# OmerShubi/DL_VQA

Hardware: AMD Instinct MI355X
Metric: VQA samples/sec (train step) (higher is better)
Workload: dtype f32; 1 GPU; VqaNet train step (fwd+softCE+bwd+Adam), batch 256/GPU, 224x224 images, 14-token questions, 1000-way head, train mode; global_batch=256, image_size=224, answers=1000, vocab=5000, parallelism=dp1

## Files before the change

dl_vqa_amd/_lib.py:

```python
from __future__ import annotations

import ctypes as C
import os

import torch

_HERE = os.path.dirname(os.path.abspath(__file__))
LIB_PATH = os.environ.get("VQA_LIB", os.path.join(_HERE, "libvqa_hip.so"))
HEADER_PATH = os.path.join(os.path.dirname(_HERE), "include", "vqa_hip.h")


def header_abi_version() -> int:
    import re
    with open(HEADER_PATH) as f:
        m = re.search(r"^#define\s+VQA_ABI_VERSION\s+(\d+)", f.read(), flags=re.M)
    if not m:
        raise VqaHipError(f"{HEADER_PATH}: no VQA_ABI_VERSION")
    return int(m.group(1))


f32p = C.c_void_p
u8p = C.c_void_p
i64p = C.c_void_p
i32, i64, f32, u64, vp = C.c_int, C.c_int64, C.c_float, C.c_uint64, C.c_void_p

PROTOTYPES = {
    "vqa_abi_version": (i32, []),
    "vqa_last_error": (C.c_char_p, []),
    "vqa_device_ok": (i32, []),
    "vqa_reload_knobs": (i32, []),
    "vqa_prof_arm": (i32, [i32, i32]),
    "vqa_prof_arm_mask": (i32, [C.c_uint32, i32]),
    "vqa_prof_read": (i32, [C.POINTER(i32), C.POINTER(f32)]),
    "vqa_prof_read_groups": (i32, [C.POINTER(i32), C.POINTER(i32), C.POINTER(i32), C.POINTER(f32), i32]),
    "vqa_gemm_workspace_bytes": (i64, [i32, i32, i32]),
    "vqa_gemm": (i32, [f32p, i64, i32, f32p, i64, i32, f32p, i64, i32, i32, i32, f32p, f32p,
                       f32p, i64, i32, i32, i32, i32, f32p, f32p, i64, i32, vp]),
    "vqa_gemm_x3": (i32, [f32p, i64, i32, f32p, i64, i32, f32p, i64, i32, i32, i32, f32p, f32p,
                       f32p, i64, i32, i32, i32, i32, f32p, f32p, i64, i32, vp]),
    "vqa_gemm_x3_workspace_bytes": (i64, [i32, i32, i32]),
    "vqa_nchw_to_nhwc4": (i32, [f32p, f32p, i32, i32, i32, i32, vp]),
    "vqa_conv_pack_weights": (i32, [f32p, f32p, f32p, i32, i32, i32, vp]),
    "vqa_conv3x3_relu_pool_fwd": (i32, [f32p, f32p, f32p, f32p, u8p, i32, i32, i32, i32, i32, i32, i32, vp]),
    "vqa_conv3x3_dgrad": (i32, [f32p, u8p, f32p, f32p, i32, i32, i32, i32, i32, i32, i32, vp]),
    "vqa_conv3x3_wgrad_workspace_bytes": (i64, [i32, i32, i32, i32, i32, i32]),
    "vqa_conv3x3_wgrad": (i32, [f32p, f32p, u8p, f32p, f32p, i32, i32, i32, i32, i32, i32, i32,
                                f32p, i64, i32, vp]),
    "vqa_convk_pack_weights": (i32, [f32p, f32p, i32, i32, i32, i32, vp]),
    "vqa_convk_unpack_wgrad": (i32, [f32p, f32p, i32, i32, i32, i32, vp]),
    "vqa_convk_im2col": (i32, [f32p, f32p, i32, i32, i32, i32, i32, i32, vp]),
    "vqa_convk_relu_pool": (i32, [f32p, f32p, u8p, i32, i32, i32, i32, vp]),
    "vqa_convk_route": (i32, [f32p, u8p, f32p, i32, i32, i32, i32, vp]),
    "vqa_convk_col2im": (i32, [f32p, f32p, i32, i32, i32, i32, i32, i32, vp]),
    "vqa_conv3x3_x3_supported": (i32, [i32, i32, i32, i32, i32]),
    "vqa_x3_split": (i32, [f32p, vp, vp, vp, i64, vp]),
    "vqa_x3_pack": (i32, [f32p, vp, i64, vp]),
    "vqa_x3_pack_pooled_grad_workspace_bytes": (i64, [i32]),
    "vqa_x3_pack_pooled_grad": (i32, [f32p, u8p, vp, f32p, i64, i32, f32p, i64, vp]),
    "vqa_conv3x3_relu_pool_fwd_x3": (i32, [vp, i32, vp, f32p, vp, i32, u8p, i32, i32, i32, i32, i32, i32, i32, vp]),
    "vqa_conv3x3_dgrad_x3": (i32, [vp, i32, u8p, vp, f32p, i32, i32, i32, i32, i32, i32, i32, vp]),
    "vqa_conv3x3_wgrad_x3_workspace_bytes": (i64, [i32, i32, i32, i32, i32, i32]),
    "vqa_conv3x3_wgrad_x3": (i32, [vp, i32, f32p, vp, u8p, f32p, f32p, i32, i32, i32, i32, i32, i32, i32,
                                   f32p, i64, i32, vp]),
    "vqa_conv0_supported": (i32, [i32, i32, i32, i32, i32]),
    "vqa_conv0_relu_pool_fwd": (i32, [vp, i32, f32p, f32p, vp, i32, u8p, i32, i32, i32, i32, i32, vp]),
    "vqa_conv0_wgrad_workspace_bytes": (i64, [i32]),
    "vqa_conv0_wgrad": (i32, [vp, i32, f32p, u8p, f32p, f32p, i32, i32, i32, i32, i32, f32p, i64, vp]),
    "vqa_conv0_wgrad_bf16": (i32, [vp, i32, vp, u8p, f32p, f32p, i32, i32, i32, i32, i32, f32p, i64, vp]),
    "vqa_conv0_dgrad_supported": (i32, [i32, i32, i32, i32, i32]),
    "vqa_conv0_dgrad": (i32, [vp, i32, u8p, f32p, vp, i32, i32, i32, i32, i32, i32, i32, vp]),
# ... 185 lines not shown
```

dl_vqa_amd/build.py:

```python
from __future__ import annotations

import os
import subprocess
import sys
from concurrent.futures import ThreadPoolExecutor

HERE = os.path.dirname(os.path.abspath(__file__))
CSRC = os.path.join(HERE, "csrc")
LIB = os.path.join(HERE, "libvqa_hip.so")
SOURCES = ([("gemm.hip", f"_p{k}", [f"-DVQA_GEMM_PART={k}"]) for k in (2, 3, 4, 5)]
           + [("gemm_x3.hip", f"_p{k}", [f"-DVQA_GEMM_PART={k}"]) for k in (1, 2, 3, 4)]
           + ["bf16.hip", ("gemm.hip", "_p1", ["-DVQA_GEMM_PART=1"]), "conv.hip", "conv_x3.hip", "conv_bf16.hip", "conv_patch_bf16.hip", "conv_patch_f32.hip", "gemm_tall_bf16.hip", "gemm.hip",
              "gemm_x3.hip", "runtime.hip", "conv0.hip", "conv0_dgrad.hip", "lstm.hip", "elementwise.hip", "conv_generic.hip", "att_score.hip", "att_apply.hip", "occlusion.hip", "faithfulness.hip", "lstm_occl.hip", "topk.hip", "preprocess.hip",
              "gather.hip", "adam.hip"])
HEADERS = ["common.hpp", "cache_load.hpp", "occl_core.hpp", "gemm_core.hpp", "gemm_epilogue.hpp", "gemm_host.hpp", "bf16_core.hpp", "x3_core.hpp", "conv_device.inc", "conv_host.inc", "conv_bf16.inc", os.path.join("..", "..", "include", "vqa_hip.h")]
FLAGS = ["-O3", "--offload-arch=gfx950", "-fPIC", "-std=c++17", "-Wno-unused-result"]


def _hipcc() -> str:
    for cand in (os.environ.get("HIPCC"), "/opt/rocm/bin/hipcc", "hipcc"):
        if cand and (os.path.isabs(cand) and os.path.exists(cand) or not os.path.isabs(cand)):
            return cand
    return "hipcc"


def _stale(target: str, deps) -> bool:
    if not os.path.exists(target):
        return True
    t = os.path.getmtime(target)
    return any(os.path.getmtime(d) > t for d in deps if os.path.exists(d))


def _deps(src: str, seen=None) -> list:
    import re
    seen = set() if seen is None else seen
    out = []
    try:
        text = open(src).read()
# ... 43 lines not shown
```

dl_vqa_amd/csrc/common.hpp:

```cpp
#pragma once
#include <hip/hip_runtime.h>
#include <stdint.h>
#include <stdio.h>
#include <string.h>

#include <type_traits>

#include "../../include/vqa_hip.h"

namespace vqa {

void set_error(const char* fmt, ...);
int check_hip(hipError_t e, const char* what);

#define VQA_REQUIRE(cond, ...)                 \
  do {                                         \
    if (!(cond)) {                             \
      ::vqa::set_error(__VA_ARGS__);           \
      return VQA_ERR_INVALID;                  \
    }                                          \
  } while (0)

int ensure_dyn_smem(const void* kernel, int bytes, const char* what);
template <class K>
// ... 28 lines not shown
}
template <class F>
static int with_int14(int v, F&& f) {
  switch (v) {
    case 1: return f(std::integral_constant<int, 1>{});
    case 2: return f(std::integral_constant<int, 2>{});
    case 3: return f(std::integral_constant<int, 3>{});
    default: return f(std::integral_constant<int, 4>{});
  }
}

template <class... P>
static inline uintptr_t ptr_bits(const P*... p) { return (uintptr_t{0} | ... | reinterpret_cast<uintptr_t>(p)); }

static inline float keep_scale(float p) { return p > 0.f ? 1.0f / (1.0f - p) : 1.0f; }

struct Knobs {
  int split_target;
  int big_tiles;
  int persistent;
  int weight_stationary;
  int wgrad_192;
  int wgrad_384;
  int conv_chunk;
  int tall_bm;
};
const Knobs& knobs();

void set_launch_tag(int tag);
struct ProfScope {
  int id;
  hipStream_t s;
  bool on;
  ProfScope(int id_, hipStream_t s_);
  ~ProfScope();
};

__device__ __forceinline__ int xcd_swizzle(int bid, int nwg) {
  const int xcd = bid & 7, q = nwg >> 3, r = nwg & 7;
  const int base = (xcd < r) ? xcd * (q + 1) : r * (q + 1) + (xcd - r) * q;
  return base + (bid >> 3);
}

__device__ __forceinline__ uint32_t mix32(uint32_t x) {
  x ^= x >> 16; x *= 0x7feb352dU; x ^= x >> 15; x *= 0x846ca68bU; x ^= x >> 16;
  return x;
// ... 60 lines not shown
```

dl_vqa_amd/csrc/conv.hip:

```cpp
#include "bf16_core.hpp"

namespace vqa {

#include "conv_device.inc"
#include "conv_host.inc"

using Cfg128 = TileCfg<128, 128, 2, 2>;
using Cfg128x64 = TileCfg<128, 64, 2, 2>;
#ifndef VQA_BIG_PF
#define VQA_BIG_PF 0
#endif
using Cfg256x128 = TileCfg<256, 128, 4, 2, 4, VQA_BIG_PF>;
using Cfg256x64 = TileCfg<256, 64, 4, 2, 4, VQA_BIG_PF>;
using Cfg64 = TileCfg<64, 64, 2, 2>;
#ifndef VQA_WGRAD_PF
#define VQA_WGRAD_PF 3
#endif
using Cfg96x128 = TileCfg<96, 128, 1, 4, 4, VQA_WGRAD_PF>;
using Cfg128W = TileCfg<128, 128, 2, 2, 4, VQA_WGRAD_PF>;
#ifndef VQA_W192_PF
#define VQA_W192_PF 3
#endif
using Cfg192x128W = TileCfg<192, 128, 2, 4, 4, VQA_W192_PF>;
using Cfg384x128W = TileCfg<384, 128, 4, 2, 4, 2>;
// ... 40 lines not shown
  const int big = (KI >= 128 && g.Co >= 128) ? 1 : 0;
  int bm = !big ? 64 : ((KI + 95) / 96 * 96 < (KI + 127) / 128 * 128 ? 96 : 128);
  {
    const int w192 = knobs().wgrad_192, w384 = knobs().wgrad_384;
    const bool can = big && KI % 192 == 0 && g.CiP % BK == 0 && g.Co % BK == 0 && 2 * g.Wp >= BK;
    if (can && (w192 >= 0 ? w192 == 1 : bm == 96)) bm = 192;
    if (can && KI % 384 == 0 && w192 != 1 && (w384 >= 0 ? w384 == 1 : true)) bm = 384;
  }
  WgradPlanF p{plan_splits(g, bm, big ? 128 : 64, BK, bm >= 192 ? 256 : 512), big, bm};
  p.bias_parts = p.splits;
  return p;
}

template <class Cfg, bool U>
static int launch_wgrad(const float* x, const float* dp, const uint8_t* am, float* slab, float* bias_slab,
                        const ConvGeom& g, const WgradPlan& p, hipStream_t s) {
  using SL = SmemLayout<Cfg, false, false>;
  WgradGeom wg{g.H, g.W, g.CiP, g.Hp, g.Wp, g.Co, g.stride, p.Mtot};
  typename WgradA<Cfg::NVA, Cfg::LT, U>::Params pa{x, wg, p.KI};
  typename WgradB<Cfg::NVB, Cfg::LT, U>::Params pb{dp, am, wg};
  return launch_kernel(conv_wgrad_kernel<Cfg, U>, {"attr(conv_wgrad)", "conv_wgrad launch"},
                       p.tiles_m * p.tiles_n * p.splits, Cfg::THREADS, SL::BYTES, s, pa, pb, slab, bias_slab, p.tiles_m,
                       p.tiles_n, p.nk, p.ks_per_split);
}

}

using namespace vqa;

extern "C" {

int vqa_nchw_to_nhwc4(const float* x, float* y, int B, int C, int H, int W, vqa_stream_t stream) {
  VQA_REQUIRE(x && y && C >= 1 && C <= 4, "vqa_nchw_to_nhwc4: C=%d must be 1..4", C);
  const int64_t HW = (int64_t)H * W, total = (int64_t)B * HW;
  int blocks = (int)((total + 255) / 256);
  if (blocks > 8192) blocks = 8192;
  hipLaunchKernelGGL(nchw_to_nhwc4_kernel, dim3(blocks), dim3(256), 0, (hipStream_t)stream, x, y, C, HW, total);
  return check_hip(hipGetLastError(), "nchw_to_nhwc4 launch");
}

int vqa_conv_pack_weights(const float* w, float* wf, float* wd, int Co, int Ci, int CiP, vqa_stream_t stream) {
  VQA_REQUIRE(w && wf && Ci <= CiP && CiP % 4 == 0, "vqa_conv_pack_weights: bad args Ci=%d CiP=%d", Ci, CiP);
  const int total = 9 * CiP * Co;
  hipLaunchKernelGGL(pack_weights_kernel, dim3((total + 255) / 256), dim3(256), 0, (hipStream_t)stream, w, wf, wd,
                     Co, Ci, CiP);
  return check_hip(hipGetLastError(), "pack_weights launch");
// ... 37 lines not shown
int64_t vqa_conv3x3_wgrad_workspace_bytes(int B, int H, int W, int CiP, int Co, int stride) {
  if (no_windows(B, H, W, stride)) return 0;
  const ConvWalk w{"vqa_conv3x3_wgrad", B, H, W, CiP, Co, stride, batch_chunk(B, H, W, CiP, Co, stride)};
  return slab_bytes(w, count_slabs(w, plan_wgrad));
}

int vqa_conv3x3_wgrad(const float* x, const float* dpooled, const uint8_t* argmax, float* dw, float* dbias, int B,
                      int H, int W, int CiP, int Ci, int Co, int stride, float* workspace, int64_t workspace_bytes,
                      int tag, vqa_stream_t stream) {
  VQA_REQUIRE(x && dpooled && argmax && dw && dbias && workspace && B > 0, "vqa_conv3x3_wgrad: null pointer");
  VQA_REQUIRE(Ci >= 1 && Ci <= CiP, "vqa_conv3x3_wgrad: Ci=%d CiP=%d", Ci, CiP);
  const ConvWalk w{"vqa_conv3x3_wgrad", B, H, W, CiP, Co, stride, batch_chunk(B, H, W, CiP, Co, stride)};
  hipStream_t s = (hipStream_t)stream;
  return wgrad_walk(
      w, plan_wgrad, 0, workspace, workspace_bytes, dw, Ci, tag, s,
      [&](const ConvChunk& c, const WgradPlanF& p, float* slab, float* bias_slab) {
        auto go = [&](auto cfg, auto uni) {
          return launch_wgrad<decltype(cfg), decltype(uni)::value>(x + c.xo, dpooled + c.po, argmax + c.po, slab, bias_slab,
                                                                   c.g, p, s);
        };
        auto go_uni = [&](auto cfg) {
          return with_flag(CiP % BK == 0 && Co % BK == 0 && 2 * c.g.Wp >= BK, [&](auto uni) { return go(cfg, uni); });
        };
        return p.bm == 384   ? go(Cfg384x128W{}, Flag<true>{})
               : p.bm == 192 ? go(Cfg192x128W{}, Flag<true>{})
               : p.bm == 96  ? go_uni(Cfg96x128{})
               : p.big       ? go_uni(Cfg128W{})
                             : go_uni(Cfg64{});
      },
      [&](const float* bias_rows, int n) { return reduce_bias_rows(bias_rows, dbias, n, Co, s); });
}

}

#ifdef VQA_DIAG
extern "C" int vqa_diag_read(unsigned long long* out8) {
  unsigned long long z[4] = {0, 0, 0, 0};
  hipDeviceSynchronize();
  if (hipMemcpyFromSymbol(out8, HIP_SYMBOL(vqa::vqa_diag_buf), sizeof(z)) != hipSuccess) return 1;
  if (hipMemcpyFromSymbol(out8 + 4, HIP_SYMBOL(vqa::vqa_diag_ld), sizeof(z)) != hipSuccess) return 1;
  if (hipMemcpyToSymbol(HIP_SYMBOL(vqa::vqa_diag_ld), z, sizeof(z)) != hipSuccess) return 1;
  return hipMemcpyToSymbol(HIP_SYMBOL(vqa::vqa_diag_buf), z, sizeof(z)) == hipSuccess ? 0 : 1;
}
#endif
```

dl_vqa_amd/csrc/conv_device.inc:

```
#ifdef VQA_EXP_NOAM
#define AM_LOAD(...) 0u
#else
#define AM_LOAD(...) buf_load4(__VA_ARGS__)
#endif

struct ConvGeom {
  int B, H, W, CiP, Co, stride, Ho, Wo, Hp, Wp;
};
static ConvGeom make_geom(int B, int H, int W, int CiP, int Co, int stride) {
  ConvGeom g{B, H, W, CiP, Co, stride, 0, 0, 0, 0};
  g.Ho = (H - 3) / stride + 1;
  g.Wo = (W - 3) / stride + 1;
  g.Hp = g.Ho / 2;
  g.Wp = g.Wo / 2;
  return g;
}

struct TapCursor {
  int tap, ch, C;
  __device__ __forceinline__ void init(int k, int C_) { C = C_; tap = k / C_; ch = k - tap * C_; }
  __device__ __forceinline__ void advance() {
    ch += BK;
    while (ch >= C) { ch -= C; ++tap; }
  }
};

// ... 521 lines not shown
    if (rc.yo + 1 == rc.Ho2 && n1 < BK) l1 += fix_img;
    const uint32_t off = kr < n1 ? lp0 : l1;
    if ((ks + 1) * BK <= q.g.Mtot) {
#pragma unroll
      for (int p = 0; p < NV; ++p) r.v[p] = buf_load16(rs, off, base + su[p]);
    } else {
      const uint32_t o2 = rc.m0 + kr < q.g.Mtot ? off + base : BUF_OOB;
#pragma unroll
      for (int p = 0; p < NV; ++p) r.v[p] = buf_load16(rs, o2, su[p]);
    }
    rc.advance();
  }
  __device__ __forceinline__ void finish(const Raw& r, float4 (&o)[NV]) const {
#pragma unroll
    for (int p = 0; p < NV; ++p) o[p] = r.v[p];
  }
};

template <int NV, int LT>
struct WgradB<NV, LT, true> {
  struct Params { const float* dp; const uint8_t* am; WgradGeom g; };
  struct Raw { float4 d[NV]; uint32_t id[NV]; uint32_t j; };
  static constexpr bool kTypeR = false;
  Params q;
  uint32_t lw0, lwE;
  uint32_t j0, win;
  int kr, n0, hw;
  RowCursor rc;
  __device__ __forceinline__ void init(const Params& q_, int n0_, int tid, int ks0) {
    q = q_; n0 = n0_;
    kr = StageMap<LT>::c_krow(tid);
    hw = __builtin_amdgcn_readfirstlane(tid >> 8);
    rc.init(ks0 * BK, q.g.Hp, q.g.Wp);
    win = (uint32_t)q.g.Co * 4u;
    lw0 = (uint32_t)(kr >> 1) * win + 16u * (uint32_t)(tid & 7);
    lwE = lw0 - (uint32_t)q.g.Wp * win;
    j0 = (uint32_t)(kr & 1);
  }
  __device__ __forceinline__ void issue(int ks, Raw& r) {
    const __amdgpu_buffer_rsrc_t rd = buf_rsrc(q.dp + n0), ra = buf_rsrc(q.am + n0, BUF_OOB >> 2);
    const int n1 = rc.Wo2 - rc.xs;
    const bool odd = rc.yo & 1;
    const int R = rc.b * rc.Ho2 + rc.yo;
    const uint32_t base = (uint32_t)((R >> 1) * q.g.Wp + (rc.xs >> 1)) * win;
    const bool second = kr >= n1;
    uint32_t off = (second && !odd ? lwE : lw0) + base;
// ... 35 lines not shown
  float cs[Cfg::TN];
#pragma unroll
  for (int j = 0; j < Cfg::TN; ++j) cs[j] = 0.f;
  if (!gemm_mainloop<Cfg, AL, BL>(
          [&](AL& al, BL& bl) {
            al.init(pa, m0, loader_tid<Cfg>(), ks0);
            bl.init(pb, n0, loader_tid<Cfg>(), ks0);
          },
          [](AL&, BL&) {}, acc, ks0, ks1, pa.g.Mtot, smem, (tc.mt == 0 && wm == 0) ? cs : nullptr))
    return;
  if (tc.mt == 0 && wm == 0) {
#pragma unroll
    for (int j = 0; j < Cfg::TN; ++j) {
      const float v = cs[j] + __shfl_xor(cs[j], 32, 64);
      const int col = n0 + acc_col<Cfg>(wn, j, lane);
      if (lane < 32 && col < pa.g.Co) bias_slab[(int64_t)split * pa.g.Co + col] = v;
    }
  }
  const int Co = pa.g.Co;
  float* out = slab + (int64_t)split * pa.KI * Co;
  store_acc_tiles<Cfg>(acc, out, Co, pa.KI, Co, m0, n0, wm, wn, lane);
}

static __global__ __launch_bounds__(256) void wgrad_reduce_kernel(const float* slab, float* dw, int splits, int KI, int CiP,
                                                           int Ci, int Co) {
  __shared__ float part[4][64];
  const int lane = threadIdx.x & 63, grp = threadIdx.x >> 6;
  const int src = blockIdx.x * 64 + lane;
  const int total = KI * Co;
  float v = 0.f;
  if (src < total)
    for (int s = grp; s < splits; s += 4) v += slab[(int64_t)s * total + src];
  part[grp][lane] = v;
  __syncthreads();
  if (grp == 0 && src < total) {
    v = (part[0][lane] + part[1][lane]) + (part[2][lane] + part[3][lane]);
    const int co = src % Co;
    const int t = src / Co;
    const int ci = t % CiP;
    const int tap = t / CiP;
    if (ci < Ci) dw[((int64_t)co * Ci + ci) * 9 + tap] = v;
  }
}

static __global__ __launch_bounds__(256) void wgrad_bias_reduce_kernel(const float* bias_slab, float* dbias, int parts, int Co) {
  __shared__ float part[8][32];
// ... 41 lines not shown
```

dl_vqa_amd/csrc/conv_patch_bf16.hip:

```cpp
#include "bf16_core.hpp"
#include <stdlib.h>

namespace vqa {

#ifdef VQA_PCONV_DIAG
#define PC_DBG(bit) (P.dbg & (bit))
#else
#define PC_DBG(bit) false
#endif

constexpr int PC_RS = 40;
constexpr int PC_TX = 32;

template <int WM_>
struct PcCfg {
  static constexpr int WM = WM_, WN = 8 / WM_;
  static constexpr int TY = 4 * WM;
  static constexpr int NSLAB = 64 * WN;
  static constexpr int NT = NSLAB / 32;
  static constexpr int PROWS = TY + 2;
  static constexpr int PATCH_BYTES = ((PROWS * PC_RS * 32 + 1023) / 1024) * 1024;
  static constexpr int PATCH_INSTR = PATCH_BYTES / 1024;
  static constexpr int PK = (PATCH_INSTR + 7) / 8;
  static constexpr int W_BYTES = 9 * NT * 1024;
// ... 6 lines not shown
  static constexpr int LDS_ALL = LDS + 8 * SCR;
  template <int EPI> static constexpr int nstores() { return EPI == 0 ? 8 : EPI == 1 ? 12 : 16; }
};

struct PcParams {
  const char* x;
  const char* x_end;
  const char* wimg;
  const float* bias;
  void* out;
  uint8_t* amax;
  const char* am_in;
  int Hq, Wq;
  int B, H, W, Cin, N;
  int Hc, Wc;
  int Hp, Wp;
  int tiles_y, tiles_x, ntiles;
  int nslabs, nslices;
  int dbg;
};

typedef __attribute__((address_space(3))) void lds_void;

typedef unsigned int pc_rsrc_t __attribute__((ext_vector_type(4)));
__device__ __forceinline__ pc_rsrc_t pc_rsrc(const void* base, uint32_t bytes = 0xffff0000u) {
  const uint64_t a = (uint64_t)base;
  pc_rsrc_t r;
  r.x = __builtin_amdgcn_readfirstlane((uint32_t)a);
  r.y = __builtin_amdgcn_readfirstlane((uint32_t)(a >> 32) & 0xffffu);
  r.z = __builtin_amdgcn_readfirstlane(bytes);
  r.w = 0x00020000u;
  return r;
}
__device__ __forceinline__ void lds_dma16(pc_rsrc_t r, const void* lds_dst, uint32_t voff, uint32_t soff) {
  const uint32_t m0v = __builtin_amdgcn_readfirstlane((uint32_t)(uintptr_t)(__attribute__((address_space(3))) const char*)lds_dst);
  uint32_t keep;
  asm volatile("s_nop 4\n\ts_mov_b32 %0, m0\n\ts_mov_b32 m0, %1\n\ts_nop 0\n\tbuffer_load_dwordx4 %2, %3, %4 offen lds\n\ts_mov_b32 m0, %0"
               : "=&s"(keep) : "s"(m0v), "v"(voff), "s"(r), "s"(soff) : "memory");
}

struct PcTile {
  int img, ty, tx;
  __device__ __forceinline__ void decode(int s, int tiles_y, int tiles_x) {
    const int per = tiles_y * tiles_x;
    img = s / per;
    const int rem = s - img * per;
    ty = rem / tiles_x;
    tx = rem - ty * tiles_x;
  }
  __device__ __forceinline__ void advance(const PcTile& d, int tiles_y, int tiles_x) {
    tx += d.tx;
    if (tx >= tiles_x) { tx -= tiles_x; ++ty; }
    ty += d.ty;
    if (ty >= tiles_y) { ty -= tiles_y; ++img; }
    img += d.img;
  }
};

__device__ __forceinline__ float4 pc_route8(float4 d, uint2 id, uint32_t j) {
  const uint32_t jj = j * 0x01010101u;
  auto bytemask = [&](uint32_t w) {
    const uint32_t q = w ^ jj;
// ... 764 lines not shown
```

dl_vqa_amd/csrc/gemm_core.hpp:

```cpp
#pragma once
#include <type_traits>
#include "common.hpp"

namespace vqa {

typedef float f32x16 __attribute__((ext_vector_type(16)));

#ifdef VQA_DIAG
static __device__ unsigned long long vqa_diag_buf[4];
static __device__ unsigned long long vqa_diag_ld[4];
#endif

#ifndef VQA_PRIO_MFMA
#define VQA_PRIO_MFMA 3
#endif
#ifndef VQA_EARLY_BARRIER
#define VQA_EARLY_BARRIER 2
#endif
#ifndef VQA_PF128
#define VQA_PF128 2
#endif
#ifndef VQA_PRIO_LOADER
#define VQA_PRIO_LOADER 0
#endif

// ... 274 lines not shown
        __syncthreads();
#elif defined(VQA_EXP_STORE_ONLY)
        stage_store_one<Cfg, AL, true>(al, rawA[d], As0 + nxt * SL::ABUF, ltid);
        stage_store_one<Cfg, BL, false>(bl, rawB[d], Bs0 + nxt * SL::BBUF, ltid);
        __syncthreads();
#else
        stage_store_one<Cfg, AL, true>(al, rawA[d], As0 + nxt * SL::ABUF, ltid);
        al.issue(ks + d + 1 + D, rawA[d]);
        stage_store_one<Cfg, BL, false>(bl, rawB[d], Bs0 + nxt * SL::BBUF, ltid);
        bl.issue(ks + d + 1 + D, rawB[d]);
        __syncthreads();
#endif
      }
    }
  }
#ifdef VQA_DIAG
  if ((threadIdx.x & 63) == 0) {
    atomicAdd(&vqa_diag_ld[0], t_st); atomicAdd(&vqa_diag_ld[1], t_is); atomicAdd(&vqa_diag_ld[2], t_ba);
    atomicAdd(&vqa_diag_ld[3], 1ULL);
  }
#endif
}

template <class Cfg, bool AR, bool BR, bool SHORT_TAIL, bool CS = false>
__device__ __forceinline__ void mfma_loop(f32x16 (&acc)[Cfg::TM][Cfg::TN], int ks0, int ks1, int Ktot,
                                          const float* smem, float* cs = nullptr) {
  using SL = SmemLayout<Cfg, AR, BR>;
  const int lane = threadIdx.x & 63, wave = threadIdx.x >> 6;
  const int wm = wave / Cfg::WAVES_N, wn = wave % Cfg::WAVES_N;
  const float* const As0 = smem;
  const float* const Bs0 = smem + 2 * SL::ABUF;
  __builtin_amdgcn_s_setprio(VQA_PRIO_MFMA);
#ifdef VQA_DIAG
  unsigned long long t_mma = 0, t_bar = 0;
  const unsigned long long t_begin = __builtin_amdgcn_s_memtime();
#endif
  __syncthreads();
  for (int ks = ks0; ks < ks1; ++ks) {
    const int cur = (ks - ks0) & 1;
    const float* const Ac = As0 + cur * SL::ABUF;
    const float* const Bc = Bs0 + cur * SL::BBUF;
#ifdef VQA_DIAG
    const unsigned long long t0 = __builtin_amdgcn_s_memtime();
#endif
#ifndef VQA_EXP_SKIP_MFMA
    if (SHORT_TAIL && Ktot - ks * BK <= 8) mma_steps<Cfg, AR, BR, 1, CS>(Ac, Bc, acc, wm, wn, lane, cs);
    else mma_steps<Cfg, AR, BR, 4, CS>(Ac, Bc, acc, wm, wn, lane, cs);
#endif
#ifdef VQA_DIAG
    const unsigned long long t1 = __builtin_amdgcn_s_memtime();
#endif
    __syncthreads();
#ifdef VQA_DIAG
    const unsigned long long t2 = __builtin_amdgcn_s_memtime();
    t_mma += t1 - t0; t_bar += t2 - t1;
#endif
  }
#ifdef VQA_DIAG
  if (lane == 0) {
    atomicAdd(&vqa_diag_buf[0], t_mma); atomicAdd(&vqa_diag_buf[1], t_bar); atomicAdd(&vqa_diag_buf[2], 1ULL);
    atomicAdd(&vqa_diag_buf[3], __builtin_amdgcn_s_memtime() - t_begin);
  }
#endif
}

template <class Cfg, bool AR, bool BR, bool CS>
__device__ __forceinline__ void mfma_loop_eb(f32x16 (&acc)[Cfg::TM][Cfg::TN], int ks0, int ks1, const float* smem,
                                             float* cs) {
  using SL = SmemLayout<Cfg, AR, BR>;
  const int lane = threadIdx.x & 63, wave = threadIdx.x >> 6;
  const int wm = wave / Cfg::WAVES_N, wn = wave % Cfg::WAVES_N;
  const int l31 = lane & 31, h = lane >> 5;
  constexpr int CSA = LdsImage<Cfg::BM>::CS, CSB = LdsImage<Cfg::BN>::CS;
  const float* const As0 = smem + (AR ? (wm * Cfg::WM + l31) * LDS_RS + 4 * h : 4 * h * CSA + wm * Cfg::WM + l31);
  const float* const Bs0 = smem + 2 * SL::ABUF + (BR ? (wn * Cfg::WN + l31) * LDS_RS + 4 * h : 4 * h * CSB + wn * Cfg::WN + l31);
  constexpr bool EB2 = Cfg::TM * Cfg::TN == 1 && VQA_EARLY_BARRIER >= 2;
  float a[EB2 ? 4 : 2][4][Cfg::TM], b[EB2 ? 4 : 2][4][Cfg::TN];
  auto fetch = [&](const float* ap, const float* bp, int t, int buf) {
#pragma unroll
    for (int i = 0; i < Cfg::TM; ++i) {
      if (AR) {
        const float4 v = *reinterpret_cast<const float4*>(ap + 32 * i * LDS_RS + 8 * t);
        a[buf][0][i] = v.x; a[buf][1][i] = v.y; a[buf][2][i] = v.z; a[buf][3][i] = v.w;
      } else {
#pragma unroll
        for (int q = 0; q < 4; ++q) a[buf][q][i] = ap[(8 * t + q) * CSA + 32 * i];
      }
    }
#pragma unroll
    for (int j = 0; j < Cfg::TN; ++j) {
      if (BR) {
        const float4 v = *reinterpret_cast<const float4*>(bp + 32 * j * LDS_RS + 8 * t);
        b[buf][0][j] = v.x; b[buf][1][j] = v.y; b[buf][2][j] = v.z; b[buf][3][j] = v.w;
      } else {
#pragma unroll
        for (int q = 0; q < 4; ++q) b[buf][q][j] = bp[(8 * t + q) * CSB + 32 * j];
      }
    }
  };
// ... 24 lines not shown
      const float* const An = As0 + (cur ^ 1) * SL::ABUF;
      const float* const Bn = Bs0 + (cur ^ 1) * SL::BBUF;
      fetch(Ac, Bc, 2, 2);
      __builtin_amdgcn_sched_barrier(0);
      mma(0);
      __builtin_amdgcn_sched_barrier(0);
      fetch(Ac, Bc, 3, 3);
      __builtin_amdgcn_sched_barrier(0);
      mma(1);
      __builtin_amdgcn_sched_barrier(0);
      __syncthreads();
      if (ks + 1 < ks1) fetch(An, Bn, 0, 0);
      __builtin_amdgcn_sched_barrier(0);
      mma(2);
      __builtin_amdgcn_sched_barrier(0);
      if (ks + 1 < ks1) fetch(An, Bn, 1, 1);
      __builtin_amdgcn_sched_barrier(0);
      mma(3);
      __builtin_amdgcn_sched_barrier(0);
    }
    return;
  }
  fetch(As0, Bs0, 0, 0);
  for (int ks = ks0; ks < ks1; ++ks) {
    const int cur = (ks - ks0) & 1;
    const float* const Ac = As0 + cur * SL::ABUF;
    const float* const Bc = Bs0 + cur * SL::BBUF;
#pragma unroll
    for (int t = 0; t < 3; ++t) {
      fetch(Ac, Bc, t + 1, (t + 1) & 1);
      __builtin_amdgcn_sched_barrier(0);
      mma(t & 1);
      __builtin_amdgcn_sched_barrier(0);
    }
    __syncthreads();
    if (ks + 1 < ks1) fetch(As0 + (cur ^ 1) * SL::ABUF, Bs0 + (cur ^ 1) * SL::BBUF, 0, 0);
    __builtin_amdgcn_sched_barrier(0);
    mma(1);
    __builtin_amdgcn_sched_barrier(0);
  }
}

template <class Cfg, class AL, class BL, bool SHORT_TAIL = false, class Init, class Done>
__device__ __forceinline__ bool gemm_mainloop(Init&& init, Done&& done, f32x16 (&acc)[Cfg::TM][Cfg::TN], int ks0,
                                              int ks1, int Ktot, float* smem, float* cs = nullptr) {
  if (is_loader_wave<Cfg>()) {
    AL al; BL bl;
    init(al, bl);
    loader_loop<Cfg>(al, bl, ks0, ks1, smem);
    done(al, bl);
    return false;
  }
#if VQA_EARLY_BARRIER && !defined(VQA_DIAG) && !defined(VQA_EXP_SKIP_MFMA)
  if (!SHORT_TAIL) {
    if (cs) mfma_loop_eb<Cfg, AL::kTypeR, BL::kTypeR, true>(acc, ks0, ks1, smem, cs);
    else mfma_loop_eb<Cfg, AL::kTypeR, BL::kTypeR, false>(acc, ks0, ks1, smem, nullptr);
    return true;
  }
#endif
  if (cs) mfma_loop<Cfg, AL::kTypeR, BL::kTypeR, SHORT_TAIL, true>(acc, ks0, ks1, Ktot, smem, cs);
  else mfma_loop<Cfg, AL::kTypeR, BL::kTypeR, SHORT_TAIL, false>(acc, ks0, ks1, Ktot, smem);
  return true;
}
// ... 160 lines not shown
```

dl_vqa_amd/csrc/runtime.hip:

```cpp
#include <stdarg.h>
#include <stdlib.h>

#include <map>
#include <mutex>
#include <set>
#include <utility>
#include <vector>

#include "gemm_host.hpp"

namespace vqa {

static thread_local char g_err[512] = "";
void set_error(const char* fmt, ...) {
  va_list ap;
  va_start(ap, fmt);
  vsnprintf(g_err, sizeof(g_err), fmt, ap);
  va_end(ap);
}
int check_hip(hipError_t e, const char* what) {
  if (e == hipSuccess) return VQA_OK;
  set_error("%s: %s", what, hipGetErrorString(e));
  return VQA_ERR_HIP;
}
// ... 39 lines not shown
  if (per_cu < 1) {
    set_error("gemm_persistent: the kernel does not fit a CU (occupancy query says %d workgroups)", per_cu);
    return -1;
  }
  const int slots = cus * (per_cu < planned_per_cu ? per_cu : planned_per_cu);
  cache[key] = slots;
  return slots;
}

static std::mutex g_knob_mu;
static Knobs g_knobs;
static bool g_knobs_read = false;
static int env_int(const char* name) {
  const char* e = getenv(name);
  return (e && *e) ? atoi(e) : -1;
}
static void read_knobs_locked() {
  g_knobs.split_target = env_int("VQA_SPLIT_TARGET");
  g_knobs.big_tiles = env_int("VQA_BIG_TILES");
  g_knobs.persistent = env_int("VQA_PERSISTENT");
  g_knobs.weight_stationary = env_int("VQA_WEIGHT_STATIONARY");
  g_knobs.wgrad_192 = env_int("VQA_WGRAD_192");
  g_knobs.wgrad_384 = env_int("VQA_WGRAD_384");
  g_knobs.conv_chunk = env_int("VQA_CONV_CHUNK");
  g_knobs.tall_bm = env_int("VQA_TALL_BM");
  g_knobs_read = true;
}
const Knobs& knobs() {
  std::lock_guard<std::mutex> lk(g_knob_mu);
  if (!g_knobs_read) read_knobs_locked();
  return g_knobs;
}

static std::mutex g_prof_mu;
static uint32_t g_prof_mask = 0;
static int g_prof_tag = -1;
static std::vector<std::pair<hipEvent_t, hipEvent_t>> g_prof_ev;
static std::vector<std::pair<int, int>> g_prof_key;
static thread_local int g_launch_tag = -1;
void set_launch_tag(int tag) { g_launch_tag = tag; }

ProfScope::ProfScope(int id_, hipStream_t s_) : id(id_), s(s_), on(false) {
  if (g_prof_mask == 0) return;
  std::lock_guard<std::mutex> lk(g_prof_mu);
  if (!((g_prof_mask >> id) & 1u) || (g_prof_tag >= 0 && g_prof_tag != g_launch_tag)) return;
  hipStreamCaptureStatus cap = hipStreamCaptureStatusNone;
// ... 154 lines not shown
```

include/vqa_hip.h:

```cpp
#ifndef VQA_HIP_H
#define VQA_HIP_H

#include <stdint.h>

#ifdef __cplusplus
extern "C" {
#endif

#define VQA_ABI_VERSION 9

#define VQA_OK 0
#define VQA_ERR_INVALID 1
#define VQA_ERR_HIP 2
#define VQA_ERR_WORKSPACE 3

typedef void* vqa_stream_t;

int vqa_abi_version(void);
const char* vqa_last_error(void);
int vqa_device_ok(void);

int vqa_reload_knobs(void);

enum {
// ... 16 lines not shown
int vqa_prof_arm(int kernel_id, int tag);
int vqa_prof_arm_mask(uint32_t mask, int tag);
int vqa_prof_read(int* launches, float* total_ms);
int vqa_prof_read_groups(int* ids, int* tags, int* launches, float* total_ms, int cap);

int64_t vqa_gemm_workspace_bytes(int M, int N, int K);
int vqa_gemm(const float* A, int64_t lda, int transA, const float* B, int64_t ldb, int transB,
             float* C, int64_t ldc, int M, int N, int K, const float* bias1, const float* bias2,
             const float* rowgroup, int64_t rg_ld, int rg_div, int rg_op, int relu, int accumulate,
             float* aux ,
             float* workspace, int64_t workspace_bytes, int tag, vqa_stream_t stream);

int vqa_nchw_to_nhwc4(const float* x_nchw, float* y_nhwc, int B, int C, int H, int W, vqa_stream_t stream);
int vqa_conv_pack_weights(const float* w, float* wf, float* wd, int Co, int Ci, int CiP, vqa_stream_t stream);
int vqa_conv3x3_relu_pool_fwd(const float* x, const float* wf, const float* bias, float* pooled,
                              uint8_t* argmax, int B, int H, int W, int CiP, int Co, int stride,
                              int tag, vqa_stream_t stream);
int vqa_conv3x3_dgrad(const float* dpooled, const uint8_t* argmax, const float* wd, float* dx, int B,
                      int H, int W, int CiP, int Co, int stride, int tag, vqa_stream_t stream);
int64_t vqa_conv3x3_wgrad_workspace_bytes(int B, int H, int W, int CiP, int Co, int stride);
int vqa_conv3x3_wgrad(const float* x, const float* dpooled, const uint8_t* argmax, float* dw,
                      float* dbias, int B, int H, int W, int CiP, int Ci, int Co, int stride,
                      float* workspace, int64_t workspace_bytes, int tag, vqa_stream_t stream);

int vqa_convk_pack_weights(const float* w, float* wk, int Co, int Ci, int CiP, int ks, vqa_stream_t stream);
int vqa_convk_unpack_wgrad(const float* dwk, float* dw, int Co, int Ci, int CiP, int ks, vqa_stream_t stream);
int vqa_convk_im2col(const float* x, float* cols, int B, int H, int W, int CiP, int ks, int stride, vqa_stream_t stream);
int vqa_convk_relu_pool(const float* y, float* pooled, uint8_t* argmax, int B, int Ho, int Wo, int Co, vqa_stream_t stream);
int vqa_convk_route(const float* dpooled, const uint8_t* argmax, float* dy, int B, int Ho, int Wo, int Co, vqa_stream_t stream);
int vqa_convk_col2im(const float* dcols, float* dx, int B, int H, int W, int CiP, int ks, int stride, vqa_stream_t stream);

int vqa_conv0_supported(int Ci, int H, int W, int Co, int stride);
int vqa_conv0_relu_pool_fwd(const void* x_nchw, int x_is_fp16 , const float* w, const float* bias, void* pooled,
                            int pooled_is_bf16 , uint8_t* argmax, int B, int Ci,
                            int H, int W, int Co, vqa_stream_t stream);
int64_t vqa_conv0_wgrad_workspace_bytes(int Co);
int vqa_conv0_wgrad(const void* x_nchw, int x_is_fp16, const float* dpooled, const uint8_t* argmax, float* dw, float* dbias,
                    int B, int Ci, int H, int W, int Co, float* workspace, int64_t workspace_bytes,
                    vqa_stream_t stream);

int vqa_conv0_wgrad_bf16(const void* x_nchw, int x_is_fp16, const void* dpooled_bf16, const uint8_t* argmax, float* dw,
                         float* dbias, int B, int Ci, int H, int W, int Co, float* workspace,
                         int64_t workspace_bytes, vqa_stream_t stream);

int vqa_conv0_dgrad_supported(int Ci, int H, int W, int Co, int stride);
int vqa_conv0_dgrad(const void* dpooled, int dpooled_is_bf16, const uint8_t* argmax, const float* w, void* dv, int dv_is_fp16,
// ... 335 lines not shown
```

Baseline: 9842 samples/s.

## Stream conv wgrad A tiles into LDS via buffer-load DMA with deeper ring

```diff
diff --git a/dl_vqa_amd/_lib.py b/dl_vqa_amd/_lib.py
--- a/dl_vqa_amd/_lib.py
+++ b/dl_vqa_amd/_lib.py
@@ -46,6 +46,7 @@
     "vqa_conv3x3_wgrad_workspace_bytes": (i64, [i32, i32, i32, i32, i32, i32]),
     "vqa_conv3x3_wgrad": (i32, [f32p, f32p, u8p, f32p, f32p, i32, i32, i32, i32, i32, i32, i32,
                                 f32p, i64, i32, vp]),
+    "vqa_conv3x3_wgrad_transport": (i32, [i32, i32, i32, i32, i32, i32]),
     "vqa_convk_pack_weights": (i32, [f32p, f32p, i32, i32, i32, i32, vp]),
     "vqa_convk_unpack_wgrad": (i32, [f32p, f32p, i32, i32, i32, i32, vp]),
     "vqa_convk_im2col": (i32, [f32p, f32p, i32, i32, i32, i32, i32, i32, vp]),
diff --git a/dl_vqa_amd/build.py b/dl_vqa_amd/build.py
--- a/dl_vqa_amd/build.py
+++ b/dl_vqa_amd/build.py
@@ -13,7 +13,7 @@
            + ["bf16.hip", ("gemm.hip", "_p1", ["-DVQA_GEMM_PART=1"]), "conv.hip", "conv_x3.hip", "conv_bf16.hip", "conv_patch_bf16.hip", "conv_patch_f32.hip", "gemm_tall_bf16.hip", "gemm.hip",
               "gemm_x3.hip", "runtime.hip", "conv0.hip", "conv0_dgrad.hip", "lstm.hip", "elementwise.hip", "conv_generic.hip", "att_score.hip", "att_apply.hip", "occlusion.hip", "faithfulness.hip", "lstm_occl.hip", "topk.hip", "preprocess.hip",
               "gather.hip", "adam.hip"])
-HEADERS = ["common.hpp", "cache_load.hpp", "occl_core.hpp", "gemm_core.hpp", "gemm_epilogue.hpp", "gemm_host.hpp", "bf16_core.hpp", "x3_core.hpp", "conv_device.inc", "conv_host.inc", "conv_bf16.inc", os.path.join("..", "..", "include", "vqa_hip.h")]
+HEADERS = ["common.hpp", "cache_load.hpp", "lds_dma.hpp", "occl_core.hpp", "gemm_core.hpp", "gemm_epilogue.hpp", "gemm_host.hpp", "bf16_core.hpp", "x3_core.hpp", "conv_device.inc", "conv_host.inc", "conv_bf16.inc", os.path.join("..", "..", "include", "vqa_hip.h")]
 FLAGS = ["-O3", "--offload-arch=gfx950", "-fPIC", "-std=c++17", "-Wno-unused-result"]
 
 
diff --git a/dl_vqa_amd/csrc/common.hpp b/dl_vqa_amd/csrc/common.hpp
--- a/dl_vqa_amd/csrc/common.hpp
+++ b/dl_vqa_amd/csrc/common.hpp
@@ -74,6 +74,7 @@
   int weight_stationary;
   int wgrad_192;
   int wgrad_384;
+  int wgrad_dma;
   int conv_chunk;
   int tall_bm;
 };
diff --git a/dl_vqa_amd/csrc/conv.hip b/dl_vqa_amd/csrc/conv.hip
--- a/dl_vqa_amd/csrc/conv.hip
+++ b/dl_vqa_amd/csrc/conv.hip
@@ -86,6 +86,39 @@
   return launch_kernel(conv_wgrad_kernel<Cfg, U>, {"attr(conv_wgrad)", "conv_wgrad launch"},
                        p.tiles_m * p.tiles_n * p.splits, Cfg::THREADS, SL::BYTES, s, pa, pb, slab, bias_slab, p.tiles_m,
                        p.tiles_n, p.nk, p.ks_per_split);
+}
+
+#ifndef VQA_WGRAD_DMA_192
+#define VQA_WGRAD_DMA_192 1
+#endif
+#ifndef VQA_WGRAD_DMA_384
+#define VQA_WGRAD_DMA_384 1
+#endif
+static bool wgrad_dma(const ConvGeom& g, const WgradPlanF& p) {
+  const int k = knobs().wgrad_dma;
+  if (k == 0 || (p.bm != 192 && p.bm != 384) || (3 * g.CiP) % p.bm != 0) return false;
+  return k > 0 || (p.bm == 192 ? VQA_WGRAD_DMA_192 : VQA_WGRAD_DMA_384) != 0;
+}
+
+#ifndef VQA_W192_SA
+#define VQA_W192_SA 4
+#endif
+#ifndef VQA_W192_D
+#define VQA_W192_D 5
+#endif
+#ifndef VQA_W384_D
+#define VQA_W384_D 3
+#endif
+template <class Cfg, int SA, int D>
+static int launch_wgrad_dma(const float* x, const float* dp, const uint8_t* am, float* slab, float* bias_slab,
+                            const ConvGeom& g, const WgradPlan& p, hipStream_t s) {
+  static_assert(DmaSmem<Cfg, SA>::BYTES <= 160 * 1024, "LDS of one workgroup");
+  WgradGeom wg{g.H, g.W, g.CiP, g.Hp, g.Wp, g.Co, g.stride, p.Mtot};
+  typename WgradA<Cfg::NVA, Cfg::LT, true>::Params pa{x, wg, p.KI};
+  typename WgradB<Cfg::NVB, Cfg::LT, true>::Params pb{dp, am, wg};
+  return launch_kernel(conv_wgrad_dma_kernel<Cfg, SA, D>, {"attr(conv_wgrad_dma)", "conv_wgrad_dma launch"},
+                       p.tiles_m * p.tiles_n * p.splits, Cfg::THREADS, DmaSmem<Cfg, SA>::BYTES, s, pa, pb,
+                       slab, bias_slab, p.tiles_m, p.tiles_n, p.nk, p.ks_per_split);
 }
 
 }
@@ -169,6 +202,12 @@
         auto go_uni = [&](auto cfg) {
           return with_flag(CiP % BK == 0 && Co % BK == 0 && 2 * c.g.Wp >= BK, [&](auto uni) { return go(cfg, uni); });
         };
+        if (wgrad_dma(c.g, p)) {
+          const float *xc = x + c.xo, *dpc = dpooled + c.po;
+          return p.bm == 384 ? launch_wgrad_dma<Cfg384x128W, 2, VQA_W384_D>(xc, dpc, argmax + c.po, slab, bias_slab, c.g, p, s)
+                             : launch_wgrad_dma<Cfg192x128W, VQA_W192_SA, VQA_W192_D>(
+                                   xc, dpc, argmax + c.po, slab, bias_slab, c.g, p, s);
+        }
         return p.bm == 384   ? go(Cfg384x128W{}, Flag<true>{})
                : p.bm == 192 ? go(Cfg192x128W{}, Flag<true>{})
                : p.bm == 96  ? go_uni(Cfg96x128{})
@@ -176,6 +215,16 @@
                              : go_uni(Cfg64{});
       },
       [&](const float* bias_rows, int n) { return reduce_bias_rows(bias_rows, dbias, n, Co, s); });
+}
+
+int vqa_conv3x3_wgrad_transport(int B, int H, int W, int CiP, int Co, int stride) {
+  VQA_REQUIRE(CiP > 0 && Co > 0 && CiP % 4 == 0 && Co % 4 == 0 && (stride == 1 || stride == 2) && !no_windows(B, H, W, stride),
+              "vqa_conv3x3_wgrad_transport: bad shape B=%d H=%d W=%d CiP=%d Co=%d stride=%d", B, H, W, CiP, Co, stride);
+  const int chunk = batch_chunk(B, H, W, CiP, Co, stride);
+  VQA_REQUIRE(chunk > 0, "vqa_conv3x3_wgrad_transport: one %dx%dx%d image reaches 4 GiB", H, W, CiP);
+  const ConvGeom g = make_geom(chunk, H, W, CiP, Co, stride);
+  const WgradPlanF p = plan_wgrad(g);
+  return p.bm | (wgrad_dma(g, p) ? VQA_WGRAD_TRANSPORT_DMA : 0);
 }
 
 }
diff --git a/dl_vqa_amd/csrc/conv_device.inc b/dl_vqa_amd/csrc/conv_device.inc
--- a/dl_vqa_amd/csrc/conv_device.inc
+++ b/dl_vqa_amd/csrc/conv_device.inc
@@ -1,7 +1,9 @@
 #ifdef VQA_EXP_NOAM
 #define AM_LOAD(...) 0u
+#define AM_LOADS 0
 #else
 #define AM_LOAD(...) buf_load4(__VA_ARGS__)
+#define AM_LOADS 1
 #endif
 
 struct ConvGeom {
@@ -569,6 +571,7 @@
   struct Params { const float* dp; const uint8_t* am; WgradGeom g; };
   struct Raw { float4 d[NV]; uint32_t id[NV]; uint32_t j; };
   static constexpr bool kTypeR = false;
+  static constexpr int kLoads = NV * (1 + AM_LOADS);
   Params q;
   uint32_t lw0, lwE;
   uint32_t j0, win;
@@ -650,6 +653,96 @@
   store_acc_tiles<Cfg>(acc, out, Co, pa.KI, Co, m0, n0, wm, wn, lane);
 }
 
+template <int BM>
+struct WgradADma {
+  static constexpr int PPW = BK / 4;
+  static constexpr int PIECES = (BM * 4 + 1023) / 1024;
+  static constexpr int OPS = PPW * PIECES;
+  static constexpr int LAST_LANES = (BM * 4 - 1024 * (PIECES - 1)) / 16;
+  static constexpr int KROW = (LdsImage<BM>::CS) * 4;
+  static_assert(BM % 4 == 0 && PIECES <= 2 && KROW % 16 == 0, "k-rows of one or two 16-byte-aligned pieces");
+  pc_rsrc_t rs;
+  uint32_t pix, row, img, rowfix, fix_img, tile0, vl;
+  int k0, Mtot;
+  bool last_on;
+  RowCursor rc;
+  template <class P>
+  __device__ __forceinline__ void init(const P& q, int i0, int wave, int lane, int ks0) {
+    rs = pc_rsrc(q.x);
+    Mtot = q.g.Mtot;
+    rc.init(ks0 * BK, q.g.Hp, q.g.Wp);
+    pix = (uint32_t)(q.g.stride * q.g.CiP) * 4u; row = (uint32_t)q.g.W * pix;
+    img = (uint32_t)(q.g.H * q.g.W * q.g.CiP) * 4u;
+    rowfix = row - (uint32_t)rc.Wo2 * pix;
+    fix_img = img - (uint32_t)rc.Ho2 * row;
+    const int ky = i0 / (3 * q.g.CiP);
+    tile0 = (uint32_t)(ky * q.g.W * q.g.CiP + (i0 - ky * 3 * q.g.CiP)) * 4u;
+    k0 = PPW * wave;
+    vl = 16u * (uint32_t)lane;
+    last_on = lane < LAST_LANES;
+  }
+  __device__ __forceinline__ void issue(int ks, float* stage, bool live) {
+    const int n1 = rc.Wo2 - rc.xs;
+    const uint32_t base = (uint32_t)rc.b * img + (uint32_t)rc.yo * row + (uint32_t)rc.xs * pix + tile0;
+    const uint32_t second = rowfix + (rc.yo + 1 == rc.Ho2 ? fix_img : 0u);
+    const bool whole = (ks + 1) * BK <= Mtot;
+    char* const dst0 = reinterpret_cast<char*>(stage);
+#pragma unroll
+    for (int i = 0; i < PPW; ++i) {
+      const int k = k0 + i;
+      const uint32_t soff = base + (uint32_t)k * pix + (k >= n1 ? second : 0u);
+      pc_rsrc_t r = rs;
+      r.z = live && (whole || rc.m0 + k < Mtot) ? rs.z : 0u;
+      char* const dst = dst0 + k * KROW;
+      if (PIECES == 2) lds_dma16(r, dst, vl, soff);
+      if (last_on) lds_dma16(r, dst + 1024 * (PIECES - 1), vl, soff + 1024u * (PIECES - 1));
+    }
+    rc.advance();
+  }
+};
+
+template <class Cfg, int SA, int D>
+__global__ __launch_bounds__(Cfg::THREADS, Cfg::MIN_WAVES)
+void conv_wgrad_dma_kernel(typename WgradA<Cfg::NVA, Cfg::LT, true>::Params pa, typename WgradB<Cfg::NVB, Cfg::LT, true>::Params pb,
+                           float* slab, float* bias_slab, int tiles_m, int tiles_n, int nk, int ks_per_split) {
+  static_assert(Cfg::LT == 256, "four loader waves");
+  extern __shared__ __attribute__((aligned(16))) float smem[];
+  const int tid = threadIdx.x, lane = tid & 63, wave = tid >> 6;
+  const int wm = wave / Cfg::WAVES_N, wn = wave % Cfg::WAVES_N;
+  const TileCoord tc = tile_coord(tiles_m, tiles_n);
+  const int m0 = tc.mt * Cfg::BM, n0 = tc.nt * Cfg::BN;
+  const int split = tc.split;
+  const int ks0 = split * ks_per_split;
+  const int ks1 = min(nk, ks0 + ks_per_split);
+  using AD = WgradADma<Cfg::BM>;
+  using BL = WgradB<Cfg::NVB, Cfg::LT, true>;
+  if (tid >= Cfg::MFMA_THREADS) {
+    const int w = __builtin_amdgcn_readfirstlane((tid >> 6) & 3);
+    AD ad; BL bl;
+    ad.init(pa, m0, w, lane, ks0);
+    bl.init(pb, n0, loader_tid<Cfg>(), ks0);
+    loader_loop_dma<Cfg, AD, BL, SA, D>(ad, bl, ks0, ks1, smem);
+    return;
+  }
+  f32x16 acc[Cfg::TM][Cfg::TN];
+  acc_zero<Cfg>(acc);
+  float cs[Cfg::TN];
+#pragma unroll
+  for (int j = 0; j < Cfg::TN; ++j) cs[j] = 0.f;
+  mfma_role_ring<Cfg, SA>(acc, ks0, ks1, pa.g.Mtot, smem, (tc.mt == 0 && wm == 0) ? cs : nullptr);
+  if (tc.mt == 0 && wm == 0) {
+#pragma unroll
+    for (int j = 0; j < Cfg::TN; ++j) {
+      const float v = cs[j] + __shfl_xor(cs[j], 32, 64);
+      const int col = n0 + acc_col<Cfg>(wn, j, lane);
+      if (lane < 32 && col < pa.g.Co) bias_slab[(int64_t)split * pa.g.Co + col] = v;
+    }
+  }
+  const int Co = pa.g.Co;
+  float* out = slab + (int64_t)split * pa.KI * Co;
+  store_acc_tiles<Cfg>(acc, out, Co, pa.KI, Co, m0, n0, wm, wn, lane);
+}
+
 static __global__ __launch_bounds__(256) void wgrad_reduce_kernel(const float* slab, float* dw, int splits, int KI, int CiP,
                                                            int Ci, int Co) {
   __shared__ float part[4][64];
diff --git a/dl_vqa_amd/csrc/conv_patch_bf16.hip b/dl_vqa_amd/csrc/conv_patch_bf16.hip
--- a/dl_vqa_amd/csrc/conv_patch_bf16.hip
+++ b/dl_vqa_amd/csrc/conv_patch_bf16.hip
@@ -1,4 +1,5 @@
 #include "bf16_core.hpp"
+#include "lds_dma.hpp"
 #include <stdlib.h>
 
 namespace vqa {
@@ -52,22 +53,6 @@
 
 typedef __attribute__((address_space(3))) void lds_void;
 
-typedef unsigned int pc_rsrc_t __attribute__((ext_vector_type(4)));
-__device__ __forceinline__ pc_rsrc_t pc_rsrc(const void* base, uint32_t bytes = 0xffff0000u) {
-  const uint64_t a = (uint64_t)base;
-  pc_rsrc_t r;
-  r.x = __builtin_amdgcn_readfirstlane((uint32_t)a);
-  r.y = __builtin_amdgcn_readfirstlane((uint32_t)(a >> 32) & 0xffffu);
-  r.z = __builtin_amdgcn_readfirstlane(bytes);
-  r.w = 0x00020000u;
-  return r;
-}
-__device__ __forceinline__ void lds_dma16(pc_rsrc_t r, const void* lds_dst, uint32_t voff, uint32_t soff) {
-  const uint32_t m0v = __builtin_amdgcn_readfirstlane((uint32_t)(uintptr_t)(__attribute__((address_space(3))) const char*)lds_dst);
-  uint32_t keep;
-  asm volatile("s_nop 4\n\ts_mov_b32 %0, m0\n\ts_mov_b32 m0, %1\n\ts_nop 0\n\tbuffer_load_dwordx4 %2, %3, %4 offen lds\n\ts_mov_b32 m0, %0"
-               : "=&s"(keep) : "s"(m0v), "v"(voff), "s"(r), "s"(soff) : "memory");
-}
 
 struct PcTile {
   int img, ty, tx;
diff --git a/dl_vqa_amd/csrc/gemm_core.hpp b/dl_vqa_amd/csrc/gemm_core.hpp
--- a/dl_vqa_amd/csrc/gemm_core.hpp
+++ b/dl_vqa_amd/csrc/gemm_core.hpp
@@ -1,6 +1,7 @@
 #pragma once
 #include <type_traits>
 #include "common.hpp"
+#include "lds_dma.hpp"
 
 namespace vqa {
 
@@ -321,14 +322,68 @@
 #endif
 }
 
-template <class Cfg, bool AR, bool BR, bool SHORT_TAIL, bool CS = false>
+__device__ __forceinline__ void lds_barrier() { asm volatile("s_waitcnt lgkmcnt(0)\n\ts_barrier" ::: "memory"); }
+template <int N> __device__ __forceinline__ void wait_vmcnt() {
+  static_assert(N >= 0 && N <= 63, "vmcnt is a 6-bit counter");
+  asm volatile("s_waitcnt vmcnt(%0)" ::"n"(N) : "memory");
+}
+template <class Cfg, int SA> struct DmaSmem {
+  using SL = SmemLayout<Cfg, false, false>;
+  static constexpr int BYTES = (SA * SL::ABUF + 2 * SL::BBUF) * 4;
+};
+template <class Cfg, class AD, class BL, int SA, int D>
+__device__ __forceinline__ void loader_loop_dma(AD& ad, BL& bl, int ks0, int ks1, float* smem) {
+  using SL = SmemLayout<Cfg, false, false>;
+  static_assert(SA >= 2 && D + 3 >= SA, "the first K-steps' waits count the prologue's B loads");
+  constexpr int NA = AD::OPS, NB = BL::kLoads;
+  constexpr int NWAIT = (SA - 2) * (NA + NB) + NB;
+  const int ltid = loader_tid<Cfg>();
+  float* const Bs0 = smem + SA * SL::ABUF;
+  typename BL::Raw rawB[D];
+#ifdef VQA_EXP_SKIP_LOAD
+  lds_barrier();
+  for (int ks = ks0; ks < ks1; ++ks) lds_barrier();
+  (void)ad; (void)bl; (void)ltid; (void)Bs0; (void)rawB;
+#else
+  #pragma unroll
+  for (int s = 0; s + 1 < SA; ++s) ad.issue(ks0 + s, smem + s * SL::ABUF, ks0 + s < ks1);
+  bl.issue(ks0, rawB[0]);
+  stage_store_one<Cfg, BL, false>(bl, rawB[0], Bs0, ltid);
+#pragma unroll
+  for (int d = 0; d < D; ++d) bl.issue(ks0 + 1 + d, rawB[d]);
+  wait_vmcnt<(SA - 2) * NA + D * NB>();
+  lds_barrier();
+  int sa = SA - 1;
+  auto step = [&](int k, int d) {
+    const int nxt = ((k - ks0) & 1) ^ 1;
+    stage_store_one<Cfg, BL, false>(bl, rawB[d], Bs0 + nxt * SL::BBUF, ltid);
+    ad.issue(k + SA - 1, smem + sa * SL::ABUF, k + SA - 1 < ks1);
+    sa = sa + 1 == SA ? 0 : sa + 1;
+    bl.issue(k + 1 + D, rawB[d]);
+    wait_vmcnt<NWAIT>();
+    lds_barrier();
+  };
+  int ks = ks0;
+  for (; ks + D <= ks1; ks += D) {
+#pragma unroll
+    for (int d = 0; d < D; ++d) step(ks + d, d);
+  }
+#pragma unroll
+  for (int d = 0; d + 1 < D; ++d)
+    if (ks + d < ks1) step(ks + d, d);
+  wait_vmcnt<0>();
+#endif
+}
+
+template <class Cfg, bool AR, bool BR, bool SHORT_TAIL, bool CS = false, int SA = 2>
 __device__ __forceinline__ void mfma_loop(f32x16 (&acc)[Cfg::TM][Cfg::TN], int ks0, int ks1, int Ktot,
                                           const float* smem, float* cs = nullptr) {
   using SL = SmemLayout<Cfg, AR, BR>;
   const int lane = threadIdx.x & 63, wave = threadIdx.x >> 6;
   const int wm = wave / Cfg::WAVES_N, wn = wave % Cfg::WAVES_N;
   const float* const As0 = smem;
-  const float* const Bs0 = smem + 2 * SL::ABUF;
+  const float* const Bs0 = smem + SA * SL::ABUF;
+  int sa = 0;
   __builtin_amdgcn_s_setprio(VQA_PRIO_MFMA);
 #ifdef VQA_DIAG
   unsigned long long t_mma = 0, t_bar = 0;
@@ -337,8 +392,9 @@
   __syncthreads();
   for (int ks = ks0; ks < ks1; ++ks) {
     const int cur = (ks - ks0) & 1;
-    const float* const Ac = As0 + cur * SL::ABUF;
+    const float* const Ac = As0 + (SA == 2 ? cur : sa) * SL::ABUF;
     const float* const Bc = Bs0 + cur * SL::BBUF;
+    if (SA != 2) sa = sa + 1 == SA ? 0 : sa + 1;
 #ifdef VQA_DIAG
     const unsigned long long t0 = __builtin_amdgcn_s_memtime();
 #endif
@@ -363,7 +419,7 @@
 #endif
 }
 
-template <class Cfg, bool AR, bool BR, bool CS>
+template <class Cfg, bool AR, bool BR, bool CS, int SA = 2>
 __device__ __forceinline__ void mfma_loop_eb(f32x16 (&acc)[Cfg::TM][Cfg::TN], int ks0, int ks1, const float* smem,
                                              float* cs) {
   using SL = SmemLayout<Cfg, AR, BR>;
@@ -372,8 +428,9 @@
   const int l31 = lane & 31, h = lane >> 5;
   constexpr int CSA = LdsImage<Cfg::BM>::CS, CSB = LdsImage<Cfg::BN>::CS;
   const float* const As0 = smem + (AR ? (wm * Cfg::WM + l31) * LDS_RS + 4 * h : 4 * h * CSA + wm * Cfg::WM + l31);
-  const float* const Bs0 = smem + 2 * SL::ABUF + (BR ? (wn * Cfg::WN + l31) * LDS_RS + 4 * h : 4 * h * CSB + wn * Cfg::WN + l31);
+  const float* const Bs0 = smem + SA * SL::ABUF + (BR ? (wn * Cfg::WN + l31) * LDS_RS + 4 * h : 4 * h * CSB + wn * Cfg::WN + l31);
   constexpr bool EB2 = Cfg::TM * Cfg::TN == 1 && VQA_EARLY_BARRIER >= 2;
+  static_assert(SA == 2 || !EB2, "an A ring of more than two stages: tiles of several MFMA tiles per wave only");
   float a[EB2 ? 4 : 2][4][Cfg::TM], b[EB2 ? 4 : 2][4][Cfg::TN];
   auto fetch = [&](const float* ap, const float* bp, int t, int buf) {
 #pragma unroll
@@ -444,10 +501,12 @@
     return;
   }
   fetch(As0, Bs0, 0, 0);
+  int sa = 0;
   for (int ks = ks0; ks < ks1; ++ks) {
     const int cur = (ks - ks0) & 1;
-    const float* const Ac = As0 + cur * SL::ABUF;
+    const float* const Ac = As0 + (SA == 2 ? cur : sa) * SL::ABUF;
     const float* const Bc = Bs0 + cur * SL::BBUF;
+    if (SA != 2) sa = sa + 1 == SA ? 0 : sa + 1;
 #pragma unroll
     for (int t = 0; t < 3; ++t) {
       fetch(Ac, Bc, t + 1, (t + 1) & 1);
@@ -456,11 +515,23 @@
       __builtin_amdgcn_sched_barrier(0);
     }
     __syncthreads();
-    if (ks + 1 < ks1) fetch(As0 + (cur ^ 1) * SL::ABUF, Bs0 + (cur ^ 1) * SL::BBUF, 0, 0);
+    if (ks + 1 < ks1) fetch(As0 + (SA == 2 ? cur ^ 1 : sa) * SL::ABUF, Bs0 + (cur ^ 1) * SL::BBUF, 0, 0);
     __builtin_amdgcn_sched_barrier(0);
     mma(1);
     __builtin_amdgcn_sched_barrier(0);
   }
+}
+
+template <class Cfg, int SA>
+__device__ __forceinline__ void mfma_role_ring(f32x16 (&acc)[Cfg::TM][Cfg::TN], int ks0, int ks1, int Ktot, const float* smem,
+                                               float* cs) {
+#if VQA_EARLY_BARRIER && !defined(VQA_DIAG) && !defined(VQA_EXP_SKIP_MFMA)
+  if (cs) mfma_loop_eb<Cfg, false, false, true, SA>(acc, ks0, ks1, smem, cs);
+  else mfma_loop_eb<Cfg, false, false, false, SA>(acc, ks0, ks1, smem, nullptr);
+#else
+  if (cs) mfma_loop<Cfg, false, false, false, true, SA>(acc, ks0, ks1, Ktot, smem, cs);
+  else mfma_loop<Cfg, false, false, false, false, SA>(acc, ks0, ks1, Ktot, smem);
+#endif
 }
 
 template <class Cfg, class AL, class BL, bool SHORT_TAIL = false, class Init, class Done>
diff --git a/dl_vqa_amd/csrc/lds_dma.hpp b/dl_vqa_amd/csrc/lds_dma.hpp
--- /dev/null
+++ b/dl_vqa_amd/csrc/lds_dma.hpp
@@ -0,0 +1,23 @@
+#pragma once
+#include "common.hpp"
+
+namespace vqa {
+
+typedef unsigned int pc_rsrc_t __attribute__((ext_vector_type(4)));
+__device__ __forceinline__ pc_rsrc_t pc_rsrc(const void* base, uint32_t bytes = 0xffff0000u) {
+  const uint64_t a = (uint64_t)base;
+  pc_rsrc_t r;
+  r.x = __builtin_amdgcn_readfirstlane((uint32_t)a);
+  r.y = __builtin_amdgcn_readfirstlane((uint32_t)(a >> 32) & 0xffffu);
+  r.z = __builtin_amdgcn_readfirstlane(bytes);
+  r.w = 0x00020000u;
+  return r;
+}
+__device__ __forceinline__ void lds_dma16(pc_rsrc_t r, const void* lds_dst, uint32_t voff, uint32_t soff) {
+  const uint32_t m0v = __builtin_amdgcn_readfirstlane((uint32_t)(uintptr_t)(__attribute__((address_space(3))) const char*)lds_dst);
+  uint32_t keep;
+  asm volatile("s_nop 4\n\ts_mov_b32 %0, m0\n\ts_mov_b32 m0, %1\n\ts_nop 0\n\tbuffer_load_dwordx4 %2, %3, %4 offen lds\n\ts_mov_b32 m0, %0"
+               : "=&s"(keep) : "s"(m0v), "v"(voff), "s"(r), "s"(soff) : "memory");
+}
+
+}
diff --git a/dl_vqa_amd/csrc/runtime.hip b/dl_vqa_amd/csrc/runtime.hip
--- a/dl_vqa_amd/csrc/runtime.hip
+++ b/dl_vqa_amd/csrc/runtime.hip
@@ -85,6 +85,7 @@
   g_knobs.weight_stationary = env_int("VQA_WEIGHT_STATIONARY");
   g_knobs.wgrad_192 = env_int("VQA_WGRAD_192");
   g_knobs.wgrad_384 = env_int("VQA_WGRAD_384");
+  g_knobs.wgrad_dma = env_int("VQA_WGRAD_DMA");
   g_knobs.conv_chunk = env_int("VQA_CONV_CHUNK");
   g_knobs.tall_bm = env_int("VQA_TALL_BM");
   g_knobs_read = true;
diff --git a/include/vqa_hip.h b/include/vqa_hip.h
--- a/include/vqa_hip.h
+++ b/include/vqa_hip.h
@@ -62,6 +62,8 @@
 int vqa_conv3x3_wgrad(const float* x, const float* dpooled, const uint8_t* argmax, float* dw,
                       float* dbias, int B, int H, int W, int CiP, int Ci, int Co, int stride,
                       float* workspace, int64_t workspace_bytes, int tag, vqa_stream_t stream);
+#define VQA_WGRAD_TRANSPORT_DMA 0x10000
+int vqa_conv3x3_wgrad_transport(int B, int H, int W, int CiP, int Co, int stride);
 
 int vqa_convk_pack_weights(const float* w, float* wk, int Co, int Ci, int CiP, int ks, vqa_stream_t stream);
 int vqa_convk_unpack_wgrad(const float* dwk, float* dw, int Co, int Ci, int CiP, int ks, vqa_stream_t stream);
```

Result: no change. 9928 samples/s (median of 6 runs) (+0.9%).
